# NeLy-EPFL/DeepFly3D

Hardware: AMD Instinct MI355X
Metric: frames/sec (7-view 2D->3D) (higher is better)
Workload: dtype f32; 1 GPU; BASELINE configs[1]: 2176 frames x 7 views 256x512x3 per GPU, 2-stack hourglass fp32, arg-max + 38-joint layout + fp64 DLT; frames_per_gpu=2176, parallelism=frame-sharded x1, one packed gather, collective_executed=False

## Files before the change

### deepfly3d_amd/csrc/hg_bt_wino_f32.h

```cpp
#pragma once
#include "hg_bt_ring_f32.h"

#ifndef WN_ABL
#define WN_ABL 0
#endif

namespace hgk {

constexpr int WN_CHUNKS = 16;
constexpr int WN_U_BYTES = WN_CHUNKS * 16 * 4 * 1024;
constexpr int WN_W3_BYTES = BRF_W3_STAGES * BR_STAGE_BYTES;
constexpr int WN_STREAM_BYTES = WN_U_BYTES + WN_W3_BYTES;
constexpr int WN_STREAM_BYTES_L2 = WN_U_BYTES + 2 * WN_W3_BYTES;
constexpr int WN_V_BYTES = 16 * 1024;
constexpr int WN_T1_OFF = 2 * WN_V_BYTES;
constexpr int WN_T1_BYTES = 2 * BR_T1_BYTES;
constexpr int WN_T2_BYTES = BT_TH * BT_TW * 512;
constexpr int WN_B3_OFF = WN_T1_OFF + WN_T1_BYTES;
constexpr int WN_RING2_OFF = WN_B3_OFF + 1024 + 512;
constexpr int WN_LDS_BYTES = WN_RING2_OFF + BR_RING_BYTES;
static_assert(WN_LDS_BYTES <= 160 * 1024, "one workgroup per CU");
static_assert(WN_T1_OFF == BR_RING_BYTES, "the W3 ring takes the V buffers' place");
static_assert(WN_T2_BYTES <= WN_T1_BYTES, "t2 lives in the t1 region");

__global__ __launch_bounds__(256) void bt_wino_pack_kernel(const float* __restrict__ w2, float* __restrict__ ustream) {
    const int idx = blockIdx.x * 256 + threadIdx.x;
    if (idx >= 128 * 128) return;
    const int co = idx >> 7, ci = idx & 127;
    double g[3][3];
#pragma unroll
    for (int ky = 0; ky < 3; ++ky)
#pragma unroll
        for (int kx = 0; kx < 3; ++kx) g[ky][kx] = (double)w2[((size_t)(ky * 3 + kx) * 128 + co) * 128 + ci];
    double t[4][3];
#pragma unroll
    for (int kx = 0; kx < 3; ++kx) {
        t[0][kx] = g[0][kx];
        t[1][kx] = 0.5 * (g[0][kx] + g[1][kx] + g[2][kx]);
        t[2][kx] = 0.5 * (g[0][kx] - g[1][kx] + g[2][kx]);
        t[3][kx] = g[2][kx];
    }
    const int c = ci >> 3, half = (ci >> 2) & 1, e = ci & 3, w = co >> 5, l31 = co & 31;
#pragma unroll
    for (int i = 0; i < 4; ++i) {
        const double u[4] = {t[i][0], 0.5 * (t[i][0] + t[i][1] + t[i][2]), 0.5 * (t[i][0] - t[i][1] + t[i][2]), t[i][2]};
#pragma unroll
        for (int j = 0; j < 4; ++j)
            ustream[((size_t)(((c * 4 + e) * 4 + w) * 4 + j) * 64 + half * 32 + l31) * 4 + i] = (float)(((i == 2) != (j == 2)) ? -u[j] : u[j]);
    }
}

__global__ __launch_bounds__(256) void bt_wino_pack_w3_kernel(const float* __restrict__ w3, unsigned char* __restrict__ stream) {
    const int idx = blockIdx.x * 256 + threadIdx.x;
    if (idx >= BRF_W3_STAGES * 512) return;
    const int k = idx >> 9, rem = idx & 511, c = rem & 3, r = rem >> 2, nh = k >> 3, k8 = k & 7;
    const int ch = 4 * (r & 31) + (r >> 5);
    *reinterpret_cast<u32x4*>(stream + (size_t)k * BR_STAGE_BYTES + br_swz(r, c)) = *reinterpret_cast<const u32x4*>(w3 + ((size_t)nh * 128 + ch) * 128 + 16 * k8 + 4 * c);
}

__device__ __forceinline__ void wn_uload4(f32x4 (&d)[4], const void* sbase, unsigned voff) {
    asm volatile("s_nop 4\n\tglobal_load_dwordx4 %0, %4, %5\n\tglobal_load_dwordx4 %1, %4, %5 offset:1024\n\t"
                 "global_load_dwordx4 %2, %4, %5 offset:2048\n\tglobal_load_dwordx4 %3, %4, %5 offset:3072"
                 : "=&v"(d[0]), "=&v"(d[1]), "=&v"(d[2]), "=&v"(d[3])
                 : "v"(voff), "s"(sbase)
                 : "memory");
}
template <int N>
__device__ __forceinline__ void wn_uwait(f32x4 (&u)[4]) {
    asm volatile("s_waitcnt vmcnt(%4)" : "+v"(u[0]), "+v"(u[1]), "+v"(u[2]), "+v"(u[3]) : "n"(N) : "memory");
}
__device__ __forceinline__ void wn_xload1(f32x4& d, const void* sbase, unsigned voff) {
    asm volatile("s_nop 4\n\tglobal_load_dwordx4 %0, %1, %2" : "=&v"(d) : "v"(voff), "s"(sbase) : "memory");
}
template <int STEP>
__device__ __forceinline__ void wn_xload4s(f32x4 (&d)[4], const void* sbase, unsigned voff) {
    asm volatile("s_nop 4\n\tglobal_load_dwordx4 %0, %4, %5\n\tglobal_load_dwordx4 %1, %4, %5 offset:%6\n\t"
                 "global_load_dwordx4 %2, %4, %5 offset:%7\n\tglobal_load_dwordx4 %3, %4, %5 offset:%8"
                 : "=&v"(d[0]), "=&v"(d[1]), "=&v"(d[2]), "=&v"(d[3])
                 : "v"(voff), "s"(sbase), "n"(STEP), "n"(2 * STEP), "n"(3 * STEP)
                 : "memory");
}
typedef float f32x2 __attribute__((ext_vector_type(2)));
__device__ __forceinline__ void wn_transform(const f32x2 (&P)[4], const f32x2 (&Q)[4], f32x2 (&VT)[4], f32x2 (&VS)[4]) {
    f32x2 T0, T1, T2, T3, S0, S1, S2, S3;
    asm volatile(
        "v_pk_add_f32 %8, %16, %20 op_sel_hi:[1,0] neg_lo:[0,1]\n\t"
        "v_pk_add_f32 %12, %16, %20 op_sel:[1,0] op_sel_hi:[1,1] neg_lo:[0,1] neg_hi:[0,1]\n\t"
        "v_pk_add_f32 %9, %17, %21 op_sel_hi:[1,0] neg_lo:[0,1]\n\t"
        "v_pk_add_f32 %13, %17, %21 op_sel:[1,0] op_sel_hi:[1,1] neg_lo:[0,1] neg_hi:[0,1]\n\t"
        "v_pk_add_f32 %10, %18, %22 op_sel_hi:[1,0] neg_lo:[0,1]\n\t"
        "v_pk_add_f32 %14, %18, %22 op_sel:[1,0] op_sel_hi:[1,1] neg_lo:[0,1] neg_hi:[0,1]\n\t"
        "v_pk_add_f32 %11, %19, %23 op_sel_hi:[1,0] neg_lo:[0,1]\n\t"
        "v_pk_add_f32 %15, %19, %23 op_sel:[1,0] op_sel_hi:[1,1] neg_lo:[0,1] neg_hi:[0,1]\n\t"
        "v_pk_add_f32 %0, %8, %10 neg_lo:[0,1] neg_hi:[0,1]\n\t"
        "v_pk_add_f32 %1, %9, %10\n\t"
        "v_pk_add_f32 %2, %9, %10 neg_lo:[0,1] neg_hi:[0,1]\n\t"
// ... 11 lines not shown
__global__ __launch_bounds__(256, 1) void bottleneck_wino_f32_kernel(BtRingArgs p) {
    static_assert(!(UP && ADD2), "the fused up-path sum is written by plain blocks");
    static_assert(!L2 || (!UP && !ADD2), "layer2 is a plain block");
    using T = float;
    constexpr int CIN = L2 ? 128 : 256, CO = 256;
    extern __shared__ __attribute__((aligned(16))) unsigned char smem[];
    unsigned char* const ring = smem;
    unsigned char* const t1_lds = smem + WN_T1_OFF;
    float* const b3_lds = reinterpret_cast<float*>(smem + WN_B3_OFF);
    float* const b2_lds = b3_lds + 256;
    const unsigned ring_addr = (unsigned)(size_t)(__attribute__((address_space(3))) unsigned char*)ring;
    const unsigned t1_addr = (unsigned)(size_t)(__attribute__((address_space(3))) unsigned char*)t1_lds;

    const int tid = threadIdx.x, lane = tid & 63;
    const int wave = __builtin_amdgcn_readfirstlane(tid >> 6);
    const int half = lane >> 5, l31 = lane & 31;
    const int tiles_x = p.W / BT_TW, tiles_y = p.H / BT_TH;
    const int ntiles = p.V * tiles_y * tiles_x;
    auto tile_of = [&](int vb, int& tx0, int& ty0, int& view) {
        const int xcd = vb & 7, q = ntiles >> 3, r = ntiles & 7;
        int b = (xcd < r ? xcd * (q + 1) : r * (q + 1) + (xcd - r) * q) + (vb >> 3);
        tx0 = (b % tiles_x) * BT_TW;
        b /= tiles_x;
        ty0 = (b % tiles_y) * BT_TH;
        view = b / tiles_y;
    };
    unsigned uoff = (unsigned)(lane * 16);
    asm volatile("" : "+v"(uoff));
    auto t1_issue = [&](int tx0, int ty0, int view) {
        int lane_ = (int)(uoff >> 4);
        asm volatile("" : "+v"(lane_));
// ... 7 lines not shown
            const int pc = wave_ + 4 * k;
            if (pc < BT_HALO / 4) {
                const int hp = 4 * pc + q;
                const int hy = hp / BT_HW, hx = hp - hy * BT_HW;
                const int y = ty0 - 1 + hy, x = tx0 - 1 + hx;
                const bool ok = (unsigned)y < (unsigned)p.H && (unsigned)x < (unsigned)p.W;
                const unsigned c16 = (unsigned)((slot ^ (hx & 15)) << 4);
                const unsigned in_view = (unsigned)((y * p.W + x) * 512) + c16;
                const unsigned char* const base = ok ? tin : zer;
                br_glds_piece64(base + (ok ? in_view : c16), t1_addr + (unsigned)(pc * 1024));
                br_glds_piece64(base + (ok ? in_view + 256u : c16), t1_addr + (unsigned)(BR_T1_BYTES + pc * 1024));
            }
        }
    };

    const unsigned char* const ubase = reinterpret_cast<const unsigned char*>(p.w2d) + (size_t)wave * 4096;
    auto uload = [&](int c, int e, f32x4 (&dst)[4]) { wn_uload4(dst, ubase + (size_t)(c * 4 + e) * 16384, uoff); };

    const int ptx = lane & 7, pkq = (lane >> 3) & 1, pe = lane >> 4;
    unsigned rd[4];
#pragma unroll
    for (int bb = 0; bb < 4; ++bb) {
        const int hx = 2 * ptx + bb, hp = (2 * wave) * BT_HW + hx;
        rd[bb] = (unsigned)(hp * 256 + ((pkq ^ (hx & 15)) << 4) + 4 * pe);
    }
    const unsigned vwr = (unsigned)(pe * 4096 + pkq * 512 + (((8 * wave + ptx) ^ (pkq << 3)) << 4));
    const unsigned vrd = (unsigned)(half * 512 + ((l31 ^ (half << 3)) << 4));
    auto vbuf_off = [](int b) { return b < 2 ? b * WN_V_BYTES : WN_RING2_OFF; };
    f32x2 tP[4], tQ[4];
    unsigned ta[4];
    auto t_addr = [&](int c) {
#pragma unroll
        for (int bb = 0; bb < 4; ++bb) ta[bb] = (rd[bb] ^ (unsigned)((c & 7) << 5)) + (t1_addr + (unsigned)((c >> 3) * BR_T1_BYTES));
    };
    auto t_read = [&](int bb) {
        typedef const __attribute__((address_space(3))) float* lds_f;
        if (WN_ABL & 512) {
            asm volatile("" : "+v"(tP[bb]), "+v"(tQ[bb]));
            return;
        }
        tP[bb] = f32x2{*(lds_f)(size_t)ta[bb], *(lds_f)(size_t)(ta[bb] + BT_HW * 256)};
        tQ[bb] = f32x2{*(lds_f)(size_t)(ta[bb] + 2 * BT_HW * 256), *(lds_f)(size_t)(ta[bb] + 3 * BT_HW * 256)};
    };
    f32x2 vt[4], vs[4];
    auto t_transform = [&](int c_next_addr) {
        wn_transform(tP, tQ, vt, vs);
        t_addr(c_next_addr);
    };
    auto v_store = [&](int buf, int j) {
        unsigned char* const dst = smem + vbuf_off(buf) + vwr;
        *reinterpret_cast<f32x2*>(dst + j * 1024) = vt[j];
        *reinterpret_cast<f32x2*>(dst + j * 1024 + 8) = vs[j];
    };
    auto t_transform_write = [&](int buf, int c_next_addr) {
        if (WN_ABL & 2048) {
#pragma unroll
            for (int j = 0; j < 4; ++j) {
                vt[j] = tP[j];
                vs[j] = tQ[j];
            }
        } else {
            wn_transform(tP, tQ, vt, vs);
        }
        t_addr(c_next_addr);
        unsigned char* const dst = smem + vbuf_off(buf) + vwr;
#pragma unroll
        for (int j = 0; j < 4; ++j) {
            if (WN_ABL & 1024) {
                asm volatile("" ::"v"(vt[j]), "v"(vs[j]));
                continue;
            }
            *reinterpret_cast<f32x2*>(dst + j * 1024) = vt[j];
            *reinterpret_cast<f32x2*>(dst + j * 1024 + 8) = vs[j];
        }
    };
    auto ring_slot = [](int k) { return (k & 7) < 4 ? (k & 7) * BR_STAGE_BYTES : WN_RING2_OFF + ((k & 7) - 4) * BR_STAGE_BYTES; };
    auto ring_issue8 = [&](int set) {
        unsigned wvoff = (unsigned)wave * 2048u + uoff;
        asm volatile("" : "+v"(wvoff));
#pragma unroll
        for (int k = 8 * set; k < 8 * set + 8; ++k)
            br_glds_stage(reinterpret_cast<const unsigned char*>(p.w2d) + WN_U_BYTES + (size_t)k * BR_STAGE_BYTES, wvoff,
                          ring_addr + (unsigned)ring_slot(k) + (unsigned)wave * 2048);
    };

#ifdef DF3D_BT_TIMING
    unsigned long long stamp_ = __builtin_amdgcn_s_memtime();
#endif
    int vb = blockIdx.x;
// ... 2 lines not shown
    t1_issue(tx0, ty0, view);
    b3_lds[tid] = L2 ? p.b3[tid] + p.bd[tid] : p.b3[tid];
    if (tid < 128) b2_lds[tid] = p.b2[tid];
    bool first = true;

#pragma unroll 1
    for (;;) {
        const int vbn = vb + (int)gridDim.x;
        const bool has_next = vbn < ntiles;
        int ntx0 = 0, nty0 = 0, nview = 0;
        if (has_next) tile_of(vbn, ntx0, nty0, nview);
        const size_t ftile = (((size_t)view * p.H + ty0 + 2 * wave) * p.W + tx0) * (CO * 4);
        const size_t htile = (((size_t)view * (p.H / 2) + ty0 / 2 + wave) * (p.W / 2) + tx0 / 2) * (CO * 4);
        const unsigned char* const xtile = reinterpret_cast<const unsigned char*>(p.in) + (L2 ? ftile / 2 : ftile);

        f32x16 acc[16];
        f32x4 ufr[4][4];
        uload(0, 0, ufr[0]);
        uload(0, 1, ufr[1]);
        uload(0, 2, ufr[2]);
        if (first) asm volatile("s_waitcnt vmcnt(12)" ::: "memory");
        first = false;
        br_barrier();
        BR_STAMP(0);
        asm volatile("" : "+v"(rd[0]), "+v"(rd[1]), "+v"(rd[2]), "+v"(rd[3]));
        t_addr(0);
#pragma unroll
        for (int g = 0; g < 4; ++g) t_read(g);
        t_transform_write(0, 1);
#pragma unroll
        for (int g = 0; g < 4; ++g) t_read(g);
        t_transform_write(1, 2);
        br_barrier();
        BR_STAMP(1);

        f32x4 vf[2][4];
        auto chunk = [&](int c, auto br_tag, auto first_tag) {
            constexpr int BR = decltype(br_tag)::value;
            constexpr bool FIRST = decltype(first_tag)::value;
            const int cn = c + 1 < WN_CHUNKS ? c + 1 : c;
            const int c2 = c + 2 < WN_CHUNKS ? c + 2 : WN_CHUNKS - 1, c3 = c + 3 < WN_CHUNKS ? c + 3 : WN_CHUNKS - 1;
            (void)c2;
            const unsigned char* const vb_ = smem + vbuf_off(BR) + vrd;
            const unsigned char* const vn_ = smem + vbuf_off((BR + 1) % 3) + vrd;
            if (FIRST) {
#pragma unroll
                for (int g = 0; g < 4; ++g) vf[0][g] = *reinterpret_cast<const f32x4*>(vb_ + g * 1024);
            }
#pragma unroll
            for (int e = 0; e < 4; ++e) {
                __builtin_amdgcn_sched_barrier(0);
                if (!(WN_ABL & 1)) {
                    wn_uwait<8>(ufr[e]);
                    if (e == 0) uload(c, 3, ufr[3]);
                    else uload(cn, e - 1, ufr[e - 1]);
                    __builtin_amdgcn_sched_barrier(0);
                }
                if (e == 2 && !(WN_ABL & 2)) {
                    if (WN_ABL & 4096) t_transform_write((BR + 2) % 3, c3);
                    else t_transform(c3);
                    __builtin_amdgcn_sched_barrier(0);
                }
#pragma unroll
                for (int g = 0; g < 4; ++g) {
                    if (e < 3) vf[(e + 1) & 1][g] = *reinterpret_cast<const f32x4*>(vb_ + (e + 1) * 4096 + g * 1024);
                    else vf[0][g] = *reinterpret_cast<const f32x4*>(vn_ + g * 1024);
                    if (e == 0 && !(WN_ABL & 2)) t_read(g);
                    if (e == 2 && !(WN_ABL & (2 | 4096 | 1024))) v_store((BR + 2) % 3, g);
#pragma unroll
                    for (int i = 0; i < 4; ++i) {
                        if (FIRST && e == 0)
                            acc[4 * i + g] = __builtin_amdgcn_mfma_f32_32x32x2f32(ufr[e][g][i], vf[e & 1][g][i], f32x16{0, 0, 0, 0, 0, 0, 0, 0, 0, 0, 0, 0, 0, 0, 0, 0}, 0, 0, 0);
                        else
                            acc[4 * i + g] = __builtin_amdgcn_mfma_f32_32x32x2f32(ufr[e][g][i], vf[e & 1][g][i], acc[4 * i + g], 0, 0, 0);
                    }
                    __builtin_amdgcn_sched_barrier(0);
                }
            }
            if (!(WN_ABL & 4)) br_barrier();
        };
        chunk(0, std::integral_constant<int, 0>{}, std::true_type{});
#pragma unroll 1
        for (int c = 1; c < WN_CHUNKS; c += 3) {
            chunk(c, std::integral_constant<int, 1>{}, std::false_type{});
            chunk(c + 1, std::integral_constant<int, 2>{}, std::false_type{});
            chunk(c + 2, std::integral_constant<int, 0>{}, std::false_type{});
        }
        if (!(WN_ABL & 1)) {
            wn_uwait<4>(ufr[0]);
            wn_uwait<0>(ufr[1]);
            wn_uwait<0>(ufr[2]);
        }

        BR_STAMP(2);
        int lane3 = (int)(uoff >> 4);
        asm volatile("" : "+v"(lane3));
        const int half3 = lane3 >> 5, l31_3 = lane3 & 31;
        const unsigned char* const wf0 = ring + br_swz(l31_3, half3);
        const unsigned char* const wf1 = ring + br_swz(l31_3, 2 + half3);
        const int py = 2 * wave + (l31_3 >> 4), px = l31_3 & 15;
        const unsigned lane_full = (unsigned)((4 * half3 * CO + 4 * l31_3) * 4);
        const unsigned lane_half = (unsigned)((2 * half3 * CO + 4 * l31_3) * 4);
        ring_issue8(0);

        if (WN_ABL & 16) {
            float keep = 0.0f;
#pragma unroll
            for (int k = 0; k < 16; ++k) keep += acc[k][0];
            *reinterpret_cast<float*>(t1_lds + lane3 * 4) = keep;
        } else {
            const int ty = l31_3 >> 3, tx = l31_3 & 7;
            const unsigned wbase = (unsigned)((32 * ty + 2 * tx) * 512 + ((((8 * wave + half3) ^ (2 * tx) ^ (ty & 1)) & 31) << 4));
#pragma unroll
            for (int q = 0; q < 4; ++q) {
                f32x4 y[2][2];
                const f32x4 bb = *reinterpret_cast<const f32x4*>(b2_lds + 32 * wave + 8 * q + 4 * half3);
#pragma unroll
                for (int e = 0; e < 4; ++e) {
                    const int r = 4 * q + e;
                    float s[2][4];
#pragma unroll
                    for (int j = 0; j < 4; ++j) {
                        const float m1 = j == 1 ? acc[4 + j][r] + bb[e] : acc[4 + j][r];
                        s[0][j] = acc[j][r] + m1 + acc[8 + j][r];
                        s[1][j] = m1 - acc[8 + j][r] - acc[12 + j][r];
                    }
#pragma unroll
                    for (int a = 0; a < 2; ++a) {
                        y[a][0][e] = br_relu(s[a][0] + s[a][1] + s[a][2]);
                        y[a][1][e] = br_relu(s[a][1] - s[a][2] - s[a][3]);
                    }
                }
#pragma unroll
                for (int a = 0; a < 2; ++a)
#pragma unroll
                    for (int bb = 0; bb < 2; ++bb)
                        *reinterpret_cast<f32x4*>(t1_lds + (wbase ^ (unsigned)(((2 * q) ^ bb) << 4)) + (16 * a + bb) * 512) = y[a][bb];
            }
        }
        BR_STAMP(3);
        br_wait_vm(0);
        br_barrier();
        f32x16 t2[4];
        {
            const unsigned rbase = (unsigned)((py * BT_TW + px) * 512 + ((half3 ^ (px & 15) ^ (wave & 1)) << 4));
#pragma unroll
            for (int m = 0; m < 4; ++m)
#pragma unroll
                for (int g = 0; g < 4; ++g) {
                    const f32x4 v = *reinterpret_cast<const f32x4*>(t1_lds + (rbase ^ (unsigned)((8 * m + 2 * g) << 4)));
#pragma unroll
                    for (int e = 0; e < 4; ++e) t2[m][4 * g + e] = v[e];
// ... 139 lines not shown
```

### deepfly3d_amd/csrc/hourglass.hip

```cpp
#include <algorithm>
#include <string>
#include <vector>

#include "common.h"
#include "hg_kernels.h"
#include "hg_bt_ring.h"
#include "hg_bt_l1.h"
#include "hg_head.h"
#include "hg_bt_ring_f32.h"
#include "hg_c1_f32.h"
#include "hg_l1_f32.h"
#include "hg_bt_wino_f32.h"
#include "hg_l1_wino_f32.h"
#include "hg_c1_res_f32.h"

using namespace hgk;

namespace {

enum StepKind { ST_STEM, ST_CONV, ST_POOL, ST_UPADD, ST_BOTTLENECK, ST_HEAD };

struct TensorDesc {
    size_t off;
    int h, w, c, pitch;
};

constexpr size_t VIRTUAL_OFF = ~size_t(0);

// ... 853 lines not shown
                                DF3D_HIP(hipFuncSetAttribute(reinterpret_cast<const void*>(conv1_ring_f32_kernel<false, 128, 128, T>), hipFuncAttributeMaxDynamicSharedMemorySize, C1_LDS_BYTES));
                            const unsigned c1_grid = (unsigned)std::min<long long>(c.M / 128, 2LL * cu_count());
                            hipLaunchKernelGGL((conv1_ring_f32_kernel<false, 128, 128, T>), dim3(c1_grid), dim3(256), C1_LDS_BYTES, s, c);
                            DF3D_LAUNCH_CHECK();
                        }
                        BtRingArgs r{};
                        r.in = a.in; r.out = a.out;
                        r.t1in = c.t1;
                        r.zeros = sb + h->zero_off;
                        r.wstream = sb + st.wstream;
                        r.b2 = a.b2; r.b3 = a.b3; r.bd = a.bd;
                        r.V = n; r.H = ti.h; r.W = ti.w;
                        if (std::is_same<T, float>::value && st.wstream_w2d >= 0) {
                            r.w2d = sb + st.wstream_w2d;
                            ScopedTimer tw(h, s, "bottleneck_wino_f32_kernel<false, false, true>", 2.0 * px * (9.0 * pl * pl + (double)pl * 2 * pl + (double)cin * 2 * pl),
                                           px * 4.0 * (cin + pl + 2.0 * pl), st.m1_elems * n * eb, 2.0 * px * (4.0 * pl * pl + (double)pl * 2 * pl + (double)cin * 2 * pl));
                            if (int rc = launch_wino_f32<false, false, true>(r, n * (ti.h / BT_TH) * (ti.w / BT_TW), s)) return rc;
                            break;
                        }
                        ScopedTimer tm(h, s, std::string("layer2_tail_f32_kernel<") + tname + ">", 2.0 * px * (9.0 * pl * pl + (double)pl * 2 * pl + (double)cin * 2 * pl), px * 4.0 * (cin + pl + 2.0 * pl), st.m1_elems * n * eb);
                        static unsigned attr_t = 0;
                        if (first_use_on_this_device(attr_t))
                            DF3D_HIP(hipFuncSetAttribute(reinterpret_cast<const void*>(layer2_tail_f32_kernel<T>), hipFuncAttributeMaxDynamicSharedMemorySize, L2F_LDS_BYTES));
                        hipLaunchKernelGGL(layer2_tail_f32_kernel<T>, dim3(n * (ti.h / BT_TH) * (ti.w / BT_TW)), dim3(256), L2F_LDS_BYTES, s, r);
                        DF3D_LAUNCH_CHECK();
                    }
                    break;
                }
                if (st.l1f) {
                    if constexpr (sizeof(T) == 4) {
                        const unsigned char* const sb = reinterpret_cast<const unsigned char*>(h->lowp) + h->stream_base();
// ... 91 lines not shown
                                    if (first_use_on_this_device(attr_c1r))
                                        DF3D_HIP(hipFuncSetAttribute(reinterpret_cast<const void*>(conv1_res_f32_kernel), hipFuncAttributeMaxDynamicSharedMemorySize, C1R_LDS_BYTES));
                                    c.wstream = reinterpret_cast<const unsigned char*>(h->lowp) + h->stream_base() + st.wstream_w2d + WN_STREAM_BYTES;
                                    hipLaunchKernelGGL(conv1_res_f32_kernel, dim3((unsigned)std::min<long long>(c.M / 128, (long long)(cu_count() & ~7))), dim3(256), C1R_LDS_BYTES, s, c);
                                }
                            } else if (a.in2)
                                hipLaunchKernelGGL((conv1_ring_f32_kernel<true, 256, 128, T>), dim3(c1_grid), dim3(256), C1_LDS_BYTES, s, c);
                            else
                                hipLaunchKernelGGL((conv1_ring_f32_kernel<false, 256, 128, T>), dim3(c1_grid), dim3(256), C1_LDS_BYTES, s, c);
                            DF3D_LAUNCH_CHECK();
                        }
                    }
                    if (split && std::is_same<T, float>::value && r.w2d) {
                        const int blocks = n * (ti.h / BT_TH) * (ti.w / BT_TW);
                        ScopedTimer tm(h, s, std::string("bottleneck_wino_f32_kernel<") + (a.in2 ? "true, false, false>" : a.add2 ? "false, true, false>" : "false, false, false>"),
                                       2.0 * px * (9.0 * pl * pl + 2.0 * pl * pl), px * eb * (cin + 2.0 * pl + pl), st.m1_elems * n * eb, 2.0 * px * (4.0 * pl * pl + 2.0 * pl * pl));
                        const int rc = a.in2 ? launch_wino_f32<true, false>(r, blocks, s) : a.add2 ? launch_wino_f32<false, true>(r, blocks, s) : launch_wino_f32<false, false>(r, blocks, s);
                        if (rc) return rc;
                        break;
                    }
                    const char* const flags2 = split ? (a.in2 ? "true, false, true, " : a.add2 ? "false, true, true, " : "false, false, true, ")
                                                     : a.in2 ? "true, false, false, " : a.add2 ? "false, true, false, " : "false, false, false, ";
                    ScopedTimer tm(h, s, eb == 2 ? std::string("bottleneck_ring_kernel<") + tname + (a.in2 ? ", true, 256, false, " : a.add2 ? ", false, 256, true, " : ", false, 256, false, ") + std::to_string(ring_mode(r, h->ring2)) + ">"
                                                 : std::string("bottleneck_ring_f32_kernel<") + flags2 + tname + ">",
                                   2.0 * px * ((split ? 0.0 : (double)cin * pl) + 9.0 * pl * pl + 2.0 * pl * pl), px * eb * (cin + 2.0 * pl + (split ? pl : 0)), st.m1_elems * n * eb);
                    const int blocks = n * (ti.h / BT_TH) * (ti.w / BT_TW);
                    int lds_bytes = BR_LDS_BYTES;
#ifdef DF3D_BT_TIMING
                    if (const char* e = getenv("BR_LDS")) lds_bytes = atoi(e);
#endif
#ifdef BR_FORCE_LDS
// ... 350 lines not shown
        h->build();
    } else if (h->stream_bytes || h->dtype == DF3D_DTYPE_F32S) {
        DF3D_CHECK_ARG((reinterpret_cast<uintptr_t>(lowp_dev) & 255) == 0, "lowp buffer must be 256-byte aligned");
        if (h->dtype == DF3D_DTYPE_F32S) {
            hipLaunchKernelGGL(f32s_presplit_kernel, dim3(1024), dim3(256), 0, df3d::as_stream(stream), reinterpret_cast<const u32x4*>(blob_dev),
                               reinterpret_cast<u32x4*>(lowp_dev), h->blob_floats / 16);
            hipLaunchKernelGGL(stem_relayout_f32s_kernel, dim3((64 * 184 + 255) / 256), dim3(256), 0, df3d::as_stream(stream), blob_dev + h->steps[0].conv.w_off,
                               reinterpret_cast<unsigned short*>(reinterpret_cast<float*>(lowp_dev) + h->steps[0].conv.w_off));
            blob_dev = reinterpret_cast<const float*>(lowp_dev);
        }
        for (const Step& st : h->steps) {
            if (st.kind == ST_HEAD && st.wstream >= 0)
                hipLaunchKernelGGL(bt_fc_pack_f32_kernel, dim3((HD_FC_STAGES_F32 * 512 + 255) / 256), dim3(256), 0, df3d::as_stream(stream),
                                   blob_dev + st.conv.w_off, reinterpret_cast<unsigned char*>(lowp_dev) + h->stream_base() + st.wstream);
            if (st.kind != ST_BOTTLENECK || st.wstream < 0) continue;
            if (st.l2f) {
                hipLaunchKernelGGL(bt_l2f_pack_kernel, dim3((L2F_NSTAGE * 512 + 255) / 256), dim3(256), 0, df3d::as_stream(stream), blob_dev + st.conv2b.w_off,
                                   blob_dev + st.conv3b.w_off, blob_dev + st.conv4b.w_off, reinterpret_cast<unsigned char*>(lowp_dev) + h->stream_base() + st.wstream);
                hipLaunchKernelGGL(bt_c1_pack_f32_kernel, dim3(((128 / 16) * 512 + 255) / 256), dim3(256), 0, df3d::as_stream(stream), blob_dev + st.conv.w_off,
                                   reinterpret_cast<unsigned char*>(lowp_dev) + h->stream_base() + st.wstream_c1, 128, 128);
                if (st.wstream_w2d >= 0 && h->dtype == DF3D_DTYPE_F32) {
                    unsigned char* const ws = reinterpret_cast<unsigned char*>(lowp_dev) + h->stream_base() + st.wstream_w2d;
                    hipLaunchKernelGGL(bt_wino_pack_kernel, dim3(128 * 128 / 256), dim3(256), 0, df3d::as_stream(stream), blob_dev + st.conv2b.w_off, reinterpret_cast<float*>(ws));
                    hipLaunchKernelGGL(bt_wino_pack_w3_kernel, dim3(BRF_W3_STAGES * 512 / 256), dim3(256), 0, df3d::as_stream(stream), blob_dev + st.conv3b.w_off, ws + WN_U_BYTES);
                    hipLaunchKernelGGL(bt_wino_pack_w3_kernel, dim3(BRF_W3_STAGES * 512 / 256), dim3(256), 0, df3d::as_stream(stream), blob_dev + st.conv4b.w_off, ws + WN_U_BYTES + WN_W3_BYTES);
                }
                continue;
            }
            if (st.l1f) {
                hipLaunchKernelGGL(bt_l1f_pack_kernel, dim3((L1F_NSTAGE * 512 + 255) / 256), dim3(256), 0, df3d::as_stream(stream), blob_dev + st.conv2b.w_off,
                                   blob_dev + st.conv3b.w_off, blob_dev + st.conv4b.w_off, reinterpret_cast<unsigned char*>(lowp_dev) + h->stream_base() + st.wstream);
                hipLaunchKernelGGL(bt_c1_pack_f32_kernel, dim3(((64 / 16) * 512 + 255) / 256), dim3(256), 0, df3d::as_stream(stream), blob_dev + st.conv.w_off,
                                   reinterpret_cast<unsigned char*>(lowp_dev) + h->stream_base() + st.wstream_c1, 64, 64);
                if (st.wstream_w2d >= 0 && h->dtype == DF3D_DTYPE_F32) {
                    unsigned char* const ws = reinterpret_cast<unsigned char*>(lowp_dev) + h->stream_base() + st.wstream_w2d;
                    hipLaunchKernelGGL(l1_wino_pack_u_kernel, dim3(64 * 64 / 256), dim3(256), 0, df3d::as_stream(stream), blob_dev + st.conv2b.w_off, reinterpret_cast<float*>(ws));
                    hipLaunchKernelGGL(l1_wino_pack_w_kernel, dim3(4 * 512 / 256), dim3(256), 0, df3d::as_stream(stream), blob_dev + st.conv3b.w_off, ws + L1W_U_BYTES);
                    hipLaunchKernelGGL(l1_wino_pack_w_kernel, dim3(4 * 512 / 256), dim3(256), 0, df3d::as_stream(stream), blob_dev + st.conv4b.w_off, ws + L1W_U_BYTES + L1W_W_BYTES);
                }
                continue;
            }
            hipLaunchKernelGGL(bt_ring_pack_f32_kernel, dim3((BRF_NSTAGE * 512 + 255) / 256), dim3(256), 0, df3d::as_stream(stream),
                               blob_dev + st.conv.w_off, blob_dev + st.conv2b.w_off, blob_dev + st.conv3b.w_off,
                               reinterpret_cast<unsigned char*>(lowp_dev) + h->stream_base() + st.wstream);
            if (st.wstream_c1 >= 0)
                hipLaunchKernelGGL(bt_c1_pack_f32_kernel, dim3((C1_NSTAGE * 512 + 255) / 256), dim3(256), 0, df3d::as_stream(stream),
                                   blob_dev + st.conv.w_off, reinterpret_cast<unsigned char*>(lowp_dev) + h->stream_base() + st.wstream_c1);
            if (st.wstream_w2d >= 0 && h->dtype == DF3D_DTYPE_F32)
            {
                unsigned char* const ws = reinterpret_cast<unsigned char*>(lowp_dev) + h->stream_base() + st.wstream_w2d;
                hipLaunchKernelGGL(bt_wino_pack_kernel, dim3(128 * 128 / 256), dim3(256), 0, df3d::as_stream(stream), blob_dev + st.conv2b.w_off, reinterpret_cast<float*>(ws));
                hipLaunchKernelGGL(bt_wino_pack_w3_kernel, dim3(BRF_W3_STAGES * 512 / 256), dim3(256), 0, df3d::as_stream(stream), blob_dev + st.conv3b.w_off, ws + WN_U_BYTES);
                hipLaunchKernelGGL(c1r_pack_kernel, dim3(C1_NSTAGE * 512 / 256), dim3(256), 0, df3d::as_stream(stream), blob_dev + st.conv.w_off, ws + WN_STREAM_BYTES);
            }
        }
        if (h->uses_zero_page)
            DF3D_HIP(hipMemsetAsync(reinterpret_cast<unsigned char*>(lowp_dev) + h->stream_base() + h->zero_off, 0, 256, df3d::as_stream(stream)));
        DF3D_LAUNCH_CHECK();
        h->lowp = lowp_dev;
    }
    h->blob = blob_caller;
    return DF3D_OK;
}

size_t df3d_hg_workspace_bytes(const df3d_hg* h, int n) {
    if (!h || n <= 0) return 0;
// ... 138 lines not shown
```

Measured before the change: 707.9 frames/s.

## Switch bottleneck 3x3 Winograd from F(2x2,3x3) to F(4x2,3x3) with 16x16 MFMAs

Replaces the 4x4-tile Winograd transform (F(2,3) in both dims) with a 6x4 tile that produces 4x2 outputs (F(4,3) horizontally, F(2,3) vertically). This lowers the multiply count per output from 4 to 3 per channel pair. The weight transform now emits six passes per chunk, with the overflow stored in the unused direct-form stage-image region, and the GEMM moves from 32x32x2 to 16x16x4 MFMAs with 48 accumulators. U loads are triple-buffered and the input/output transforms are rewritten. In exchange it costs more registers, larger transform arithmetic and worse numeric conditioning (division by 15, factors of 8).

```diff
diff --git a/deepfly3d_amd/csrc/hg_bt_wino_f32.h b/deepfly3d_amd/csrc/hg_bt_wino_f32.h
--- a/deepfly3d_amd/csrc/hg_bt_wino_f32.h
+++ b/deepfly3d_amd/csrc/hg_bt_wino_f32.h
@@ -8,22 +8,33 @@
 namespace hgk {
 
 constexpr int WN_CHUNKS = 16;
-constexpr int WN_U_BYTES = WN_CHUNKS * 16 * 4 * 1024;
+constexpr int WN_PASSES = 6;
+#ifndef WN_UBUF
+#define WN_UBUF 3
+#endif
+constexpr int WN_PASS_BYTES = 4 * 4 * 1024;
+constexpr int WN_U_BYTES = 64 * WN_PASS_BYTES;
+constexpr int WN_U2_BYTES = (WN_CHUNKS * WN_PASSES - 64) * WN_PASS_BYTES;
 constexpr int WN_W3_BYTES = BRF_W3_STAGES * BR_STAGE_BYTES;
 constexpr int WN_STREAM_BYTES = WN_U_BYTES + WN_W3_BYTES;
 constexpr int WN_STREAM_BYTES_L2 = WN_U_BYTES + 2 * WN_W3_BYTES;
-constexpr int WN_V_BYTES = 16 * 1024;
-constexpr int WN_T1_OFF = 2 * WN_V_BYTES;
+constexpr int WN_V_BYTES = 12 * 1024;
+constexpr int WN_T1_OFF = BR_RING_BYTES;
 constexpr int WN_T1_BYTES = 2 * BR_T1_BYTES;
 constexpr int WN_T2_BYTES = BT_TH * BT_TW * 512;
 constexpr int WN_B3_OFF = WN_T1_OFF + WN_T1_BYTES;
 constexpr int WN_RING2_OFF = WN_B3_OFF + 1024 + 512;
 constexpr int WN_LDS_BYTES = WN_RING2_OFF + BR_RING_BYTES;
 static_assert(WN_LDS_BYTES <= 160 * 1024, "one workgroup per CU");
-static_assert(WN_T1_OFF == BR_RING_BYTES, "the W3 ring takes the V buffers' place");
+static_assert(WN_PASSES % WN_UBUF == 0 && WN_UBUF >= 2, "a chunk's passes use the same buffers in every chunk");
+static_assert(WN_V_BYTES <= BR_RING_BYTES / 2, "V buffers 0, 1 in the W3 ring's slots 0 .. 3, buffer 2 in slots 4 .. 7");
 static_assert(WN_T2_BYTES <= WN_T1_BYTES, "t2 lives in the t1 region");
-
-__global__ __launch_bounds__(256) void bt_wino_pack_kernel(const float* __restrict__ w2, float* __restrict__ ustream) {
+static_assert(WN_U2_BYTES <= BRF_NSTAGE * BR_STAGE_BYTES, "U's second part fits the direct-form stage images");
+
+__host__ __device__ constexpr int wn_row(int pg, int q4) { return pg >= 3 ? 3 - (q4 & 1) : (q4 & 1); }
+__host__ __device__ constexpr int wn_col(int pg, int q4) { return 2 * (pg % 3) + (q4 >> 1); }
+
+__global__ __launch_bounds__(256) void bt_wino_pack_kernel(const float* __restrict__ w2, float* __restrict__ ustream, float* __restrict__ ustream2) {
     const int idx = blockIdx.x * 256 + threadIdx.x;
     if (idx >= 128 * 128) return;
     const int co = idx >> 7, ci = idx & 127;
@@ -40,16 +51,26 @@
         t[2][kx] = 0.5 * (g[0][kx] - g[1][kx] + g[2][kx]);
         t[3][kx] = g[2][kx];
     }
-    const int c = ci >> 3, half = (ci >> 2) & 1, e = ci & 3, w = co >> 5, l31 = co & 31;
-#pragma unroll
-    for (int i = 0; i < 4; ++i) {
-        const double u[4] = {t[i][0], 0.5 * (t[i][0] + t[i][1] + t[i][2]), 0.5 * (t[i][0] - t[i][1] + t[i][2]), t[i][2]};
-#pragma unroll
-        for (int j = 0; j < 4; ++j)
-            ustream[((size_t)(((c * 4 + e) * 4 + w) * 4 + j) * 64 + half * 32 + l31) * 4 + i] = (float)(((i == 2) != (j == 2)) ? -u[j] : u[j]);
-    }
-}
-
+    const int c = ci >> 3, s = (ci >> 2) & 1, k = ci & 3, w = co >> 5, m = (co >> 4) & 1, r = co & 15;
+#pragma unroll
+    for (int pg = 0; pg < 6; ++pg)
+#pragma unroll
+        for (int q4 = 0; q4 < 4; ++q4) {
+            const double* const x = t[wn_row(pg, q4)];
+            double u;
+            switch (wn_col(pg, q4)) {
+                case 0: u = x[0]; break;
+                case 1: u = (x[0] + x[1] + x[2]) / 3.0; break;
+                case 2: u = (-x[0] + x[1] - x[2]) / 3.0; break;
+                case 3: u = -(16.0 * x[0] + 8.0 * x[1] + 4.0 * x[2]) / 15.0; break;
+                case 4: u = (x[0] - 2.0 * x[1] + 4.0 * x[2]) / 15.0; break;
+                default: u = x[2]; break;
+            }
+            const int P = 6 * c + 3 * s + (pg >> 1);
+            const size_t off = ((size_t)((P & 63) * 4 + w) * 4 + (pg & 1) * 2 + m) * 256 + (r + 16 * k) * 4 + q4;
+            (P < 64 ? ustream : ustream2)[off] = (float)u;
+        }
+}
 __global__ __launch_bounds__(256) void bt_wino_pack_w3_kernel(const float* __restrict__ w3, unsigned char* __restrict__ stream) {
     const int idx = blockIdx.x * 256 + threadIdx.x;
     if (idx >= BRF_W3_STAGES * 512) return;
@@ -80,6 +101,7 @@
                  : "v"(voff), "s"(sbase), "n"(STEP), "n"(2 * STEP), "n"(3 * STEP)
                  : "memory");
 }
+
 typedef float f32x2 __attribute__((ext_vector_type(2)));
 __device__ __forceinline__ void wn_transform(const f32x2 (&P)[4], const f32x2 (&Q)[4], f32x2 (&VT)[4], f32x2 (&VS)[4]) {
     f32x2 T0, T1, T2, T3, S0, S1, S2, S3;
@@ -121,7 +143,6 @@
 
     const int tid = threadIdx.x, lane = tid & 63;
     const int wave = __builtin_amdgcn_readfirstlane(tid >> 6);
-    const int half = lane >> 5, l31 = lane & 31;
     const int tiles_x = p.W / BT_TW, tiles_y = p.H / BT_TH;
     const int ntiles = p.V * tiles_y * tiles_x;
     auto tile_of = [&](int vb, int& tx0, int& ty0, int& view) {
@@ -159,65 +180,86 @@
         }
     };
 
+
     const unsigned char* const ubase = reinterpret_cast<const unsigned char*>(p.w2d) + (size_t)wave * 4096;
-    auto uload = [&](int c, int e, f32x4 (&dst)[4]) { wn_uload4(dst, ubase + (size_t)(c * 4 + e) * 16384, uoff); };
-
-    const int ptx = lane & 7, pkq = (lane >> 3) & 1, pe = lane >> 4;
-    unsigned rd[4];
-#pragma unroll
-    for (int bb = 0; bb < 4; ++bb) {
-        const int hx = 2 * ptx + bb, hp = (2 * wave) * BT_HW + hx;
-        rd[bb] = (unsigned)(hp * 256 + ((pkq ^ (hx & 15)) << 4) + 4 * pe);
-    }
-    const unsigned vwr = (unsigned)(pe * 4096 + pkq * 512 + (((8 * wave + ptx) ^ (pkq << 3)) << 4));
-    const unsigned vrd = (unsigned)(half * 512 + ((l31 ^ (half << 3)) << 4));
-    auto vbuf_off = [](int b) { return b < 2 ? b * WN_V_BYTES : WN_RING2_OFF; };
-    f32x2 tP[4], tQ[4];
-    unsigned ta[4];
+    const unsigned char* const ubase2 = reinterpret_cast<const unsigned char*>(p.wstream) + (size_t)wave * 4096 - (size_t)64 * WN_PASS_BYTES;
+    auto uload = [&](int c, int e, f32x4 (&dst)[4]) {
+        const int P = WN_PASSES * c + e;
+        wn_uload4(dst, (P < 64 ? ubase : ubase2) + (size_t)P * WN_PASS_BYTES, uoff);
+    };
+
+    const int wh = wave & 1;
+    unsigned rd[6], vwr, vrd;
+    auto lane_consts = [&]() {
+        int l = (int)(uoff >> 4);
+        asm volatile("" : "+v"(l));
+        const int ppc = l & 3, pte = (l >> 2) & 3, pkq = (l >> 4) & 1, ppr = 2 * (wave >> 1) + (l >> 5);
+#pragma unroll
+        for (int col = 0; col < 6; ++col) {
+            const int hx = 4 * ppc + col, hp = (2 * ppr + wh) * BT_HW + hx;
+            rd[col] = (unsigned)(hp * 256 + ((pkq ^ (hx & 15)) << 4) + 4 * pte);
+        }
+        vwr = (unsigned)(((pkq * 6 + 3 * wh) * 4 + pte) * 256 + (((4 * ppr + ppc) ^ (4 * pte)) << 4));
+        vrd = (unsigned)((l >> 4) * 256 + (((l & 15) ^ (4 * (l >> 4))) << 4));
+    };
+    auto vbuf_off = [](int b) { return b == 0 ? 0 : b == 1 ? BR_RING_BYTES / 2 : WN_RING2_OFF; };
+    const f32x2 cw2 = {-1.0f, wh ? 0.0f : 1.0f}, cw0 = {0.0f, wh ? -1.0f : 0.0f};
+    float tR[6][3];
+    unsigned ta[6];
     auto t_addr = [&](int c) {
 #pragma unroll
-        for (int bb = 0; bb < 4; ++bb) ta[bb] = (rd[bb] ^ (unsigned)((c & 7) << 5)) + (t1_addr + (unsigned)((c >> 3) * BR_T1_BYTES));
-    };
-    auto t_read = [&](int bb) {
+        for (int col = 0; col < 6; ++col) ta[col] = (rd[col] ^ (unsigned)((c & 7) << 5)) + (t1_addr + (unsigned)((c >> 3) * BR_T1_BYTES));
+    };
+    auto t_read = [&](int col) {
         typedef const __attribute__((address_space(3))) float* lds_f;
         if (WN_ABL & 512) {
-            asm volatile("" : "+v"(tP[bb]), "+v"(tQ[bb]));
+            asm volatile("" : "+v"(tR[col][0]), "+v"(tR[col][1]), "+v"(tR[col][2]));
             return;
         }
-        tP[bb] = f32x2{*(lds_f)(size_t)ta[bb], *(lds_f)(size_t)(ta[bb] + BT_HW * 256)};
-        tQ[bb] = f32x2{*(lds_f)(size_t)(ta[bb] + 2 * BT_HW * 256), *(lds_f)(size_t)(ta[bb] + 3 * BT_HW * 256)};
-    };
-    f32x2 vt[4], vs[4];
+#pragma unroll
+        for (int t = 0; t < 3; ++t) tR[col][t] = *(lds_f)(size_t)(ta[col] + t * BT_HW * 256);
+    };
+    f32x4 vo[3];
     auto t_transform = [&](int c_next_addr) {
-        wn_transform(tP, tQ, vt, vs);
+        f32x2 x[6];
+#pragma unroll
+        for (int col = 0; col < 6; ++col) {
+            const f32x2 P = {tR[col][0], tR[col][1]};
+            if (WN_ABL & 2048) {
+                x[col] = P;
+                continue;
+            }
+            x[col] = cw0 * f32x2{tR[col][0], tR[col][0]} + (cw2 * f32x2{tR[col][2], tR[col][2]} + P);
+        }
+        f32x2 v[6];
+        if (WN_ABL & 2048) {
+#pragma unroll
+            for (int j = 0; j < 6; ++j) v[j] = x[j];
+        } else {
+            const f32x2 h = {0.5f, 0.5f}, two = {2.0f, 2.0f};
+            const f32x2 d13 = x[3] - x[1], d24 = x[4] - x[2];
+            v[0] = h * d13 + (((x[0] + x[4]) - two * x[2]) + d13);
+            v[1] = h * x[3] + (two * x[3] + (h * x[2] + (x[4] - x[1])));
+            v[2] = h * x[3] + (((x[4] + x[1]) - two * x[2]) - h * x[2]);
+            v[3] = two * (x[3] - x[1]) + d24;
+            v[4] = h * (x[1] - x[3]) + d24;
+            v[5] = h * d24 + (((x[5] + x[1]) - two * x[3]) + d24);
+        }
+#pragma unroll
+        for (int jp = 0; jp < 3; ++jp) vo[jp] = f32x4{v[2 * jp][0], v[2 * jp][1], v[2 * jp + 1][0], v[2 * jp + 1][1]};
         t_addr(c_next_addr);
     };
-    auto v_store = [&](int buf, int j) {
-        unsigned char* const dst = smem + vbuf_off(buf) + vwr;
-        *reinterpret_cast<f32x2*>(dst + j * 1024) = vt[j];
-        *reinterpret_cast<f32x2*>(dst + j * 1024 + 8) = vs[j];
+    auto v_store = [&](int buf, int jp) {
+        if (WN_ABL & 1024) {
+            asm volatile("" ::"v"(vo[jp]));
+            return;
+        }
+        *reinterpret_cast<f32x4*>(smem + vbuf_off(buf) + vwr + jp * 1024) = vo[jp];
     };
     auto t_transform_write = [&](int buf, int c_next_addr) {
-        if (WN_ABL & 2048) {
-#pragma unroll
-            for (int j = 0; j < 4; ++j) {
-                vt[j] = tP[j];
-                vs[j] = tQ[j];
-            }
-        } else {
-            wn_transform(tP, tQ, vt, vs);
-        }
-        t_addr(c_next_addr);
-        unsigned char* const dst = smem + vbuf_off(buf) + vwr;
-#pragma unroll
-        for (int j = 0; j < 4; ++j) {
-            if (WN_ABL & 1024) {
-                asm volatile("" ::"v"(vt[j]), "v"(vs[j]));
-                continue;
-            }
-            *reinterpret_cast<f32x2*>(dst + j * 1024) = vt[j];
-            *reinterpret_cast<f32x2*>(dst + j * 1024 + 8) = vs[j];
-        }
+        t_transform(c_next_addr);
+#pragma unroll
+        for (int jp = 0; jp < 3; ++jp) v_store(buf, jp);
     };
     auto ring_slot = [](int k) { return (k & 7) < 4 ? (k & 7) * BR_STAGE_BYTES : WN_RING2_OFF + ((k & 7) - 4) * BR_STAGE_BYTES; };
     auto ring_issue8 = [&](int set) {
@@ -250,65 +292,69 @@
         const size_t htile = (((size_t)view * (p.H / 2) + ty0 / 2 + wave) * (p.W / 2) + tx0 / 2) * (CO * 4);
         const unsigned char* const xtile = reinterpret_cast<const unsigned char*>(p.in) + (L2 ? ftile / 2 : ftile);
 
-        f32x16 acc[16];
-        f32x4 ufr[4][4];
-        uload(0, 0, ufr[0]);
-        uload(0, 1, ufr[1]);
-        uload(0, 2, ufr[2]);
-        if (first) asm volatile("s_waitcnt vmcnt(12)" ::: "memory");
+        f32x4 acc[48];
+        f32x4 ufr[WN_UBUF][4];
+#pragma unroll
+        for (int e = 0; e < WN_UBUF - 1; ++e) uload(0, e, ufr[e]);
+        if (first) asm volatile("s_waitcnt vmcnt(%0)" ::"n"(4 * (WN_UBUF - 1)) : "memory");
         first = false;
         br_barrier();
         BR_STAMP(0);
-        asm volatile("" : "+v"(rd[0]), "+v"(rd[1]), "+v"(rd[2]), "+v"(rd[3]));
+        lane_consts();
         t_addr(0);
 #pragma unroll
-        for (int g = 0; g < 4; ++g) t_read(g);
+        for (int col = 0; col < 6; ++col) t_read(col);
         t_transform_write(0, 1);
 #pragma unroll
-        for (int g = 0; g < 4; ++g) t_read(g);
+        for (int col = 0; col < 6; ++col) t_read(col);
         t_transform_write(1, 2);
         br_barrier();
         BR_STAMP(1);
 
-        f32x4 vf[2][4];
+        f32x4 vf[2][2];
         auto chunk = [&](int c, auto br_tag, auto first_tag) {
             constexpr int BR = decltype(br_tag)::value;
             constexpr bool FIRST = decltype(first_tag)::value;
             const int cn = c + 1 < WN_CHUNKS ? c + 1 : c;
-            const int c2 = c + 2 < WN_CHUNKS ? c + 2 : WN_CHUNKS - 1, c3 = c + 3 < WN_CHUNKS ? c + 3 : WN_CHUNKS - 1;
-            (void)c2;
+            const int c3 = c + 3 < WN_CHUNKS ? c + 3 : WN_CHUNKS - 1;
             const unsigned char* const vb_ = smem + vbuf_off(BR) + vrd;
             const unsigned char* const vn_ = smem + vbuf_off((BR + 1) % 3) + vrd;
             if (FIRST) {
 #pragma unroll
-                for (int g = 0; g < 4; ++g) vf[0][g] = *reinterpret_cast<const f32x4*>(vb_ + g * 1024);
-            }
-#pragma unroll
-            for (int e = 0; e < 4; ++e) {
+                for (int g = 0; g < 2; ++g) vf[0][g] = *reinterpret_cast<const f32x4*>(vb_ + g * 1024);
+            }
+#pragma unroll
+            for (int e = 0; e < WN_PASSES; ++e) {
+                const int pp = e % 3;
                 __builtin_amdgcn_sched_barrier(0);
                 if (!(WN_ABL & 1)) {
-                    wn_uwait<8>(ufr[e]);
-                    if (e == 0) uload(c, 3, ufr[3]);
-                    else uload(cn, e - 1, ufr[e - 1]);
+                    wn_uwait<4 * (WN_UBUF - 2)>(ufr[e % WN_UBUF]);
+                    const int eu = e + WN_UBUF - 1;
+                    if (eu < WN_PASSES) uload(c, eu, ufr[eu % WN_UBUF]);
+                    else uload(cn, eu - WN_PASSES, ufr[eu % WN_UBUF]);
                     __builtin_amdgcn_sched_barrier(0);
                 }
-                if (e == 2 && !(WN_ABL & 2)) {
+                if (e == 3 && !(WN_ABL & 2)) {
                     if (WN_ABL & 4096) t_transform_write((BR + 2) % 3, c3);
                     else t_transform(c3);
                     __builtin_amdgcn_sched_barrier(0);
                 }
 #pragma unroll
                 for (int g = 0; g < 4; ++g) {
-                    if (e < 3) vf[(e + 1) & 1][g] = *reinterpret_cast<const f32x4*>(vb_ + (e + 1) * 4096 + g * 1024);
-                    else vf[0][g] = *reinterpret_cast<const f32x4*>(vn_ + g * 1024);
-                    if (e == 0 && !(WN_ABL & 2)) t_read(g);
-                    if (e == 2 && !(WN_ABL & (2 | 4096 | 1024))) v_store((BR + 2) % 3, g);
-#pragma unroll
-                    for (int i = 0; i < 4; ++i) {
-                        if (FIRST && e == 0)
-                            acc[4 * i + g] = __builtin_amdgcn_mfma_f32_32x32x2f32(ufr[e][g][i], vf[e & 1][g][i], f32x16{0, 0, 0, 0, 0, 0, 0, 0, 0, 0, 0, 0, 0, 0, 0, 0}, 0, 0, 0);
+                    if (g < 2) {
+                        const int en = e + 1, sn = en / 3, ppn = en % 3;
+                        if (e < WN_PASSES - 1) vf[en & 1][g] = *reinterpret_cast<const f32x4*>(vb_ + (sn * 6 + 2 * ppn + g) * 1024);
+                        else vf[0][g] = *reinterpret_cast<const f32x4*>(vn_ + g * 1024);
+                    }
+                    if (e < 2 && g < 3 && !(WN_ABL & 2)) t_read(3 * e + g);
+                    if (e == 3 && g < 3 && !(WN_ABL & (2 | 4096))) v_store((BR + 2) % 3, g);
+                    const int pgl = g >> 1, m = g & 1, ai = ((2 * pp + pgl) * 2 + m) * 4;
+#pragma unroll
+                    for (int q4 = 0; q4 < 4; ++q4) {
+                        if (FIRST && e < 3)
+                            acc[ai + q4] = __builtin_amdgcn_mfma_f32_16x16x4f32(ufr[e % WN_UBUF][2 * pgl + m][q4], vf[e & 1][pgl][q4], f32x4{0.0f, 0.0f, 0.0f, 0.0f}, 0, 0, 0);
                         else
-                            acc[4 * i + g] = __builtin_amdgcn_mfma_f32_32x32x2f32(ufr[e][g][i], vf[e & 1][g][i], acc[4 * i + g], 0, 0, 0);
+                            acc[ai + q4] = __builtin_amdgcn_mfma_f32_16x16x4f32(ufr[e % WN_UBUF][2 * pgl + m][q4], vf[e & 1][pgl][q4], acc[ai + q4], 0, 0, 0);
                     }
                     __builtin_amdgcn_sched_barrier(0);
                 }
@@ -323,9 +369,8 @@
             chunk(c + 2, std::integral_constant<int, 0>{}, std::false_type{});
         }
         if (!(WN_ABL & 1)) {
-            wn_uwait<4>(ufr[0]);
-            wn_uwait<0>(ufr[1]);
-            wn_uwait<0>(ufr[2]);
+#pragma unroll
+            for (int e = 0; e < WN_UBUF - 1; ++e) wn_uwait<0>(ufr[e]);
         }
 
         BR_STAMP(2);
@@ -342,36 +387,45 @@
         if (WN_ABL & 16) {
             float keep = 0.0f;
 #pragma unroll
-            for (int k = 0; k < 16; ++k) keep += acc[k][0];
+            for (int k = 0; k < 48; ++k) keep += acc[k][0];
             *reinterpret_cast<float*>(t1_lds + lane3 * 4) = keep;
         } else {
-            const int ty = l31_3 >> 3, tx = l31_3 & 7;
-            const unsigned wbase = (unsigned)((32 * ty + 2 * tx) * 512 + ((((8 * wave + half3) ^ (2 * tx) ^ (ty & 1)) & 31) << 4));
-#pragma unroll
-            for (int q = 0; q < 4; ++q) {
-                f32x4 y[2][2];
-                const f32x4 bb = *reinterpret_cast<const f32x4*>(b2_lds + 32 * wave + 8 * q + 4 * half3);
-#pragma unroll
-                for (int e = 0; e < 4; ++e) {
-                    const int r = 4 * q + e;
-                    float s[2][4];
-#pragma unroll
-                    for (int j = 0; j < 4; ++j) {
-                        const float m1 = j == 1 ? acc[4 + j][r] + bb[e] : acc[4 + j][r];
-                        s[0][j] = acc[j][r] + m1 + acc[8 + j][r];
-                        s[1][j] = m1 - acc[8 + j][r] - acc[12 + j][r];
+            const int q3 = lane3 >> 4, opr = (lane3 & 15) >> 2, opc = lane3 & 3;
+#pragma unroll
+            for (int m = 0; m < 2; ++m) {
+                f32x4 y[2][4];
+                const f32x4 bb = *reinterpret_cast<const f32x4*>(b2_lds + 32 * wave + 16 * m + 4 * q3);
+#pragma unroll
+                for (int reg = 0; reg < 4; ++reg) {
+                    float M[4][6];
+#pragma unroll
+                    for (int pg = 0; pg < 6; ++pg)
+#pragma unroll
+                        for (int q4 = 0; q4 < 4; ++q4) M[wn_row(pg, q4)][wn_col(pg, q4)] = acc[(pg * 2 + m) * 4 + q4][reg];
+                    M[1][1] += bb[reg];
+                    float s[2][6];
+#pragma unroll
+                    for (int j = 0; j < 6; ++j) {
+                        s[0][j] = M[0][j] + M[1][j] + M[2][j];
+                        s[1][j] = M[1][j] - M[2][j] - M[3][j];
                     }
 #pragma unroll
                     for (int a = 0; a < 2; ++a) {
-                        y[a][0][e] = br_relu(s[a][0] + s[a][1] + s[a][2]);
-                        y[a][1][e] = br_relu(s[a][1] - s[a][2] - s[a][3]);
+                        const float sa = s[a][1] + s[a][2], sb = s[a][1] - s[a][2];
+                        y[a][0][reg] = br_relu(s[a][0] + sa + s[a][3] + s[a][4]);
+                        y[a][1][reg] = br_relu(sb + 0.5f * s[a][3] - 2.0f * s[a][4]);
+                        y[a][2][reg] = br_relu(sa + 0.25f * s[a][3] + 4.0f * s[a][4]);
+                        y[a][3][reg] = br_relu(sb + 0.125f * s[a][3] - 8.0f * s[a][4] + s[a][5]);
                     }
                 }
+                const int ch = 8 * wave + 4 * m + q3;
 #pragma unroll
                 for (int a = 0; a < 2; ++a)
 #pragma unroll
-                    for (int bb = 0; bb < 2; ++bb)
-                        *reinterpret_cast<f32x4*>(t1_lds + (wbase ^ (unsigned)(((2 * q) ^ bb) << 4)) + (16 * a + bb) * 512) = y[a][bb];
+                    for (int b = 0; b < 4; ++b) {
+                        const int yy = 2 * opr + a, xx = 4 * opc + b;
+                        *reinterpret_cast<f32x4*>(t1_lds + (yy * BT_TW + xx) * 512 + (((ch ^ (xx & 15) ^ (opr & 1)) & 31) << 4)) = y[a][b];
+                    }
             }
         }
         BR_STAMP(3);
diff --git a/deepfly3d_amd/csrc/hourglass.hip b/deepfly3d_amd/csrc/hourglass.hip
--- a/deepfly3d_amd/csrc/hourglass.hip
+++ b/deepfly3d_amd/csrc/hourglass.hip
@@ -12,6 +12,7 @@
 #include "hg_l1_f32.h"
 #include "hg_bt_wino_f32.h"
 #include "hg_l1_wino_f32.h"
+static_assert(hgk::WN_U2_BYTES <= hgk::L2F_NSTAGE * hgk::BR_STAGE_BYTES, "layer2: U's second part fits the direct-form stage images");
 #include "hg_c1_res_f32.h"
 
 using namespace hgk;
@@ -895,7 +896,7 @@
                         if (std::is_same<T, float>::value && st.wstream_w2d >= 0) {
                             r.w2d = sb + st.wstream_w2d;
                             ScopedTimer tw(h, s, "bottleneck_wino_f32_kernel<false, false, true>", 2.0 * px * (9.0 * pl * pl + (double)pl * 2 * pl + (double)cin * 2 * pl),
-                                           px * 4.0 * (cin + pl + 2.0 * pl), st.m1_elems * n * eb, 2.0 * px * (4.0 * pl * pl + (double)pl * 2 * pl + (double)cin * 2 * pl));
+                                           px * 4.0 * (cin + pl + 2.0 * pl), st.m1_elems * n * eb, 2.0 * px * (3.0 * pl * pl + (double)pl * 2 * pl + (double)cin * 2 * pl));
                             if (int rc = launch_wino_f32<false, false, true>(r, n * (ti.h / BT_TH) * (ti.w / BT_TW), s)) return rc;
                             break;
                         }
@@ -1017,7 +1018,7 @@
                     if (split && std::is_same<T, float>::value && r.w2d) {
                         const int blocks = n * (ti.h / BT_TH) * (ti.w / BT_TW);
                         ScopedTimer tm(h, s, std::string("bottleneck_wino_f32_kernel<") + (a.in2 ? "true, false, false>" : a.add2 ? "false, true, false>" : "false, false, false>"),
-                                       2.0 * px * (9.0 * pl * pl + 2.0 * pl * pl), px * eb * (cin + 2.0 * pl + pl), st.m1_elems * n * eb, 2.0 * px * (4.0 * pl * pl + 2.0 * pl * pl));
+                                       2.0 * px * (9.0 * pl * pl + 2.0 * pl * pl), px * eb * (cin + 2.0 * pl + pl), st.m1_elems * n * eb, 2.0 * px * (3.0 * pl * pl + 2.0 * pl * pl));
                         const int rc = a.in2 ? launch_wino_f32<true, false>(r, blocks, s) : a.add2 ? launch_wino_f32<false, true>(r, blocks, s) : launch_wino_f32<false, false>(r, blocks, s);
                         if (rc) return rc;
                         break;
@@ -1398,14 +1399,17 @@
                 hipLaunchKernelGGL(bt_fc_pack_f32_kernel, dim3((HD_FC_STAGES_F32 * 512 + 255) / 256), dim3(256), 0, df3d::as_stream(stream),
                                    blob_dev + st.conv.w_off, reinterpret_cast<unsigned char*>(lowp_dev) + h->stream_base() + st.wstream);
             if (st.kind != ST_BOTTLENECK || st.wstream < 0) continue;
+            const bool wino_f32 = st.wstream_w2d >= 0 && h->dtype == DF3D_DTYPE_F32;
             if (st.l2f) {
-                hipLaunchKernelGGL(bt_l2f_pack_kernel, dim3((L2F_NSTAGE * 512 + 255) / 256), dim3(256), 0, df3d::as_stream(stream), blob_dev + st.conv2b.w_off,
-                                   blob_dev + st.conv3b.w_off, blob_dev + st.conv4b.w_off, reinterpret_cast<unsigned char*>(lowp_dev) + h->stream_base() + st.wstream);
+                if (!wino_f32)
+                    hipLaunchKernelGGL(bt_l2f_pack_kernel, dim3((L2F_NSTAGE * 512 + 255) / 256), dim3(256), 0, df3d::as_stream(stream), blob_dev + st.conv2b.w_off,
+                                       blob_dev + st.conv3b.w_off, blob_dev + st.conv4b.w_off, reinterpret_cast<unsigned char*>(lowp_dev) + h->stream_base() + st.wstream);
                 hipLaunchKernelGGL(bt_c1_pack_f32_kernel, dim3(((128 / 16) * 512 + 255) / 256), dim3(256), 0, df3d::as_stream(stream), blob_dev + st.conv.w_off,
                                    reinterpret_cast<unsigned char*>(lowp_dev) + h->stream_base() + st.wstream_c1, 128, 128);
-                if (st.wstream_w2d >= 0 && h->dtype == DF3D_DTYPE_F32) {
+                if (wino_f32) {
                     unsigned char* const ws = reinterpret_cast<unsigned char*>(lowp_dev) + h->stream_base() + st.wstream_w2d;
-                    hipLaunchKernelGGL(bt_wino_pack_kernel, dim3(128 * 128 / 256), dim3(256), 0, df3d::as_stream(stream), blob_dev + st.conv2b.w_off, reinterpret_cast<float*>(ws));
+                    hipLaunchKernelGGL(bt_wino_pack_kernel, dim3(128 * 128 / 256), dim3(256), 0, df3d::as_stream(stream), blob_dev + st.conv2b.w_off, reinterpret_cast<float*>(ws),
+                                       reinterpret_cast<float*>(reinterpret_cast<unsigned char*>(lowp_dev) + h->stream_base() + st.wstream));
                     hipLaunchKernelGGL(bt_wino_pack_w3_kernel, dim3(BRF_W3_STAGES * 512 / 256), dim3(256), 0, df3d::as_stream(stream), blob_dev + st.conv3b.w_off, ws + WN_U_BYTES);
                     hipLaunchKernelGGL(bt_wino_pack_w3_kernel, dim3(BRF_W3_STAGES * 512 / 256), dim3(256), 0, df3d::as_stream(stream), blob_dev + st.conv4b.w_off, ws + WN_U_BYTES + WN_W3_BYTES);
                 }
@@ -1424,16 +1428,18 @@
                 }
                 continue;
             }
-            hipLaunchKernelGGL(bt_ring_pack_f32_kernel, dim3((BRF_NSTAGE * 512 + 255) / 256), dim3(256), 0, df3d::as_stream(stream),
-                               blob_dev + st.conv.w_off, blob_dev + st.conv2b.w_off, blob_dev + st.conv3b.w_off,
-                               reinterpret_cast<unsigned char*>(lowp_dev) + h->stream_base() + st.wstream);
+            if (!wino_f32)
+                hipLaunchKernelGGL(bt_ring_pack_f32_kernel, dim3((BRF_NSTAGE * 512 + 255) / 256), dim3(256), 0, df3d::as_stream(stream),
+                                   blob_dev + st.conv.w_off, blob_dev + st.conv2b.w_off, blob_dev + st.conv3b.w_off,
+                                   reinterpret_cast<unsigned char*>(lowp_dev) + h->stream_base() + st.wstream);
             if (st.wstream_c1 >= 0)
                 hipLaunchKernelGGL(bt_c1_pack_f32_kernel, dim3((C1_NSTAGE * 512 + 255) / 256), dim3(256), 0, df3d::as_stream(stream),
                                    blob_dev + st.conv.w_off, reinterpret_cast<unsigned char*>(lowp_dev) + h->stream_base() + st.wstream_c1);
-            if (st.wstream_w2d >= 0 && h->dtype == DF3D_DTYPE_F32)
+            if (wino_f32)
             {
                 unsigned char* const ws = reinterpret_cast<unsigned char*>(lowp_dev) + h->stream_base() + st.wstream_w2d;
-                hipLaunchKernelGGL(bt_wino_pack_kernel, dim3(128 * 128 / 256), dim3(256), 0, df3d::as_stream(stream), blob_dev + st.conv2b.w_off, reinterpret_cast<float*>(ws));
+                hipLaunchKernelGGL(bt_wino_pack_kernel, dim3(128 * 128 / 256), dim3(256), 0, df3d::as_stream(stream), blob_dev + st.conv2b.w_off, reinterpret_cast<float*>(ws),
+                                   reinterpret_cast<float*>(reinterpret_cast<unsigned char*>(lowp_dev) + h->stream_base() + st.wstream));
                 hipLaunchKernelGGL(bt_wino_pack_w3_kernel, dim3(BRF_W3_STAGES * 512 / 256), dim3(256), 0, df3d::as_stream(stream), blob_dev + st.conv3b.w_off, ws + WN_U_BYTES);
                 hipLaunchKernelGGL(c1r_pack_kernel, dim3(C1_NSTAGE * 512 / 256), dim3(256), 0, df3d::as_stream(stream), blob_dev + st.conv.w_off, ws + WN_STREAM_BYTES);
             }
```

After: 738.8 frames/s, median of 6. 1.04x the previous value.
